# google/TensorNetwork

Measured on NVIDIA H100. Metric: pairwise contractions/s, higher is better.
Workload: dtype bf16

## Files before the change

### include/tnb200.h

```cpp
#ifndef TNB200_H_
#define TNB200_H_

#include <stdint.h>

#if defined(TNB200_BUILD)
#define TNB200_API __attribute__((visibility("default")))
#else
#define TNB200_API
#endif

#ifdef __cplusplus
extern "C" {
#endif

#define TNB200_MAX_NDIM 16
#define TNB200_ABI_VERSION 1

typedef enum {
  TNB200_OK = 0,
  TNB200_ERR_INVALID = -1,
  TNB200_ERR_DTYPE = -2,
  TNB200_ERR_CUDA = -3,
  TNB200_ERR_UNSUPPORTED = -4,
  TNB200_ERR_NOCONV = -5
// ... 76 lines not shown
                     int32_t axis1, int32_t axis2, void* stream);
TNB200_API int32_t tnb200_diagflat(const tnb200_tensor_t* a, const tnb200_tensor_t* c, int64_t k,
                        void* stream);

TNB200_API int32_t tnb200_svd(const tnb200_tensor_t* a, const tnb200_tensor_t* u, const tnb200_tensor_t* s,
                   const tnb200_tensor_t* vh, int32_t* info_dev, void* stream);
TNB200_API int32_t tnb200_svd_truncation_count(const tnb200_tensor_t* s, int64_t max_singular_values,
                                    int32_t use_error, double max_truncation_error,
                                    int32_t relative, int64_t* keep_dev, void* stream);

TNB200_API int32_t tnb200_eigh(const tnb200_tensor_t* a, const tnb200_tensor_t* w, const tnb200_tensor_t* v,
                               int32_t* info_dev, void* stream);

TNB200_API int32_t tnb200_arnoldi_orth(const tnb200_tensor_t* v, int32_t j, const tnb200_tensor_t* w, void* h_dev,
                                       void* stream);

TNB200_API int32_t tnb200_qr(const tnb200_tensor_t* a, const tnb200_tensor_t* q, const tnb200_tensor_t* r,
                  int32_t non_negative_diagonal, void* stream);

TNB200_API int32_t tnb200_lu_factor(const tnb200_tensor_t* a, const tnb200_tensor_t* lu, int32_t* piv_dev,
                                    int32_t* info_dev, void* stream);
TNB200_API int32_t tnb200_inv(const tnb200_tensor_t* a, const tnb200_tensor_t* x, int32_t* info_dev, void* stream);

TNB200_API int32_t tnb200_blocksparse_tensordot(const void* a_data, const void* b_data, void* c_data,
                                     int32_t dtype, int32_t nsect, const int64_t* dims_dev,
                                     const int64_t* a_map_dev, const int64_t* a_off_dev,
                                     const int64_t* b_map_dev, const int64_t* b_off_dev,
                                     const int64_t* c_map_dev, const int64_t* c_off_dev,
                                     int64_t max_m, int64_t max_n, int32_t conj_b, void* stream);

TNB200_API int32_t tnb200_svd_batched(const void* a_data, int32_t dtype, int32_t nprob, const int64_t* dims_dev,
                                      const int64_t* a_off_dev, void* u_data, const int64_t* u_off_dev, void* s_data,
                                      const int64_t* s_off_dev, void* vh_data, const int64_t* vh_off_dev,
                                      int64_t max_m, int64_t max_n, int32_t* status_dev, void* stream);

TNB200_API int32_t tnb200_blocksparse_maps(int32_t nlegs, const int64_t* dims, const int64_t* charges_dev, const int64_t* leg_off,
                                           const int32_t* order, int32_t partition, int32_t split, int64_t modulus, int64_t shift,
                                           int32_t nbins, const int64_t* tables_dev, int64_t nnz, int64_t* map_dev, void* stream);

TNB200_API int32_t tnb200_gather(const void* src, const int64_t* idx_dev, void* dst, int64_t n, int32_t dtype,
                                 int32_t scatter, void* stream);

typedef struct {
  tnb200_tensor_t a, b, c;
  int32_t naxes, nbatch;
  int32_t axes_a[TNB200_MAX_NDIM], axes_b[TNB200_MAX_NDIM];
  int32_t batch_a[TNB200_MAX_NDIM], batch_b[TNB200_MAX_NDIM];
  int32_t dep_a, dep_b;
} tnb200_chain_step_t;
TNB200_API int32_t tnb200_chain_create(int32_t nsteps, const tnb200_chain_step_t* steps, int32_t* first_unsupported,
                                       void** handle);
TNB200_API int32_t tnb200_chain_launch(void* handle, void* stream);
TNB200_API int32_t tnb200_chain_destroy(void* handle);

TNB200_API int32_t tnb200_thin_run_create(int32_t nsteps, const tnb200_chain_step_t* steps, int32_t* first_unsupported,
                                          void** handle);
TNB200_API int32_t tnb200_thin_run_launch(void* handle, void* stream);
TNB200_API int32_t tnb200_thin_run_destroy(void* handle);

#ifdef __cplusplus
}
#endif
#endif
```

### tensornetwork_b200/_lib.py

```python
import ctypes
import os

MAX_NDIM = 16
LIB_PATH = os.path.join(os.path.dirname(os.path.abspath(__file__)), "lib", "libtnb200.so")

F64, F32, F16, BF16, C64, C128, I32, I64, BOOL = range(9)
OK, ERR_INVALID, ERR_DTYPE, ERR_CUDA, ERR_UNSUPPORTED, ERR_NOCONV = 0, -1, -2, -3, -4, -5
ADD, SUB, MUL, DIV, POW = range(5)
CONJ, SQRT, ABS, NEG, EXP, LOG, SIN, COS, SIGN, REAL, IMAG = range(11)
LT, LE, GT, GE = range(4)
CONJ_A, CONJ_B = 1, 2
MATH_DEFAULT, MATH_STRICT, MATH_SIMT = 0 << 4, 1 << 4, 2 << 4


class TensorDesc(ctypes.Structure):
  _fields_ = [("data", ctypes.c_void_p), ("dtype", ctypes.c_int32), ("ndim", ctypes.c_int32),
              ("shape", ctypes.c_int64 * MAX_NDIM), ("stride", ctypes.c_int64 * MAX_NDIM)]


class ChainStep(ctypes.Structure):
  _fields_ = [("a", TensorDesc), ("b", TensorDesc), ("c", TensorDesc), ("naxes", ctypes.c_int32), ("nbatch", ctypes.c_int32),
              ("axes_a", ctypes.c_int32 * MAX_NDIM), ("axes_b", ctypes.c_int32 * MAX_NDIM),
              ("batch_a", ctypes.c_int32 * MAX_NDIM), ("batch_b", ctypes.c_int32 * MAX_NDIM),
              ("dep_a", ctypes.c_int32), ("dep_b", ctypes.c_int32)]


_P = ctypes.POINTER(TensorDesc)
_i32, _i64, _u64, _dbl, _vp = (ctypes.c_int32, ctypes.c_int64, ctypes.c_uint64, ctypes.c_double,
                               ctypes.c_void_p)
_pi32 = ctypes.POINTER(ctypes.c_int32)

SIGNATURES = {
    "tnb200_last_error": (ctypes.c_char_p, []),
    "tnb200_abi_version": (_i32, []),
    "tnb200_device_info": (_i32, [_pi32, _pi32, _pi32, ctypes.POINTER(_i64)]),
    "tnb200_last_kernel": (ctypes.c_char_p, []),
    "tnb200_launch_count": (_i64, []),
    "tnb200_tensordot": (_i32, [_P, _P, _P, _i32, _pi32, _pi32, _i32, _pi32, _pi32, _i32, _vp]),
    "tnb200_copy": (_i32, [_P, _P, _i32, _vp]),
    "tnb200_binary": (_i32, [_i32, _P, _P, _P, _vp]),
    "tnb200_unary": (_i32, [_i32, _P, _P, _vp]),
    "tnb200_affine_inplace": (_i32, [_P, _dbl, _dbl, _dbl, _dbl, _vp]),
    "tnb200_scale_by_device_scalar": (_i32, [_P, _vp, _i32, _i32, _vp]),
    "tnb200_axpy": (_i32, [_P, _P, _dbl, _dbl, _vp, _dbl, _vp]),
    "tnb200_fill": (_i32, [_P, _dbl, _dbl, _vp]),
    "tnb200_compare": (_i32, [_i32, _P, _P, _P, _vp]),
    "tnb200_index_update": (_i32, [_P, _P, _dbl, _dbl, _vp, _i32, _P, _vp]),
    "tnb200_eye": (_i32, [_P, _i64, _vp]),
    "tnb200_randn": (_i32, [_P, _u64, _vp]),
    "tnb200_uniform": (_i32, [_P, _dbl, _dbl, _u64, _vp]),
    "tnb200_norm": (_i32, [_P, _vp, _vp]),
    "tnb200_dot": (_i32, [_P, _P, _i32, _vp, _vp]),
    "tnb200_sum": (_i32, [_P, _P, _i32, _pi32, _vp]),
    "tnb200_trace": (_i32, [_P, _P, _i64, _i32, _i32, _vp]),
    "tnb200_diagflat": (_i32, [_P, _P, _i64, _vp]),
    "tnb200_svd": (_i32, [_P, _P, _P, _P, _vp, _vp]),
    "tnb200_svd_truncation_count": (_i32, [_P, _i64, _i32, _dbl, _i32, _vp, _vp]),
    "tnb200_eigh": (_i32, [_P, _P, _P, _vp, _vp]),
    "tnb200_arnoldi_orth": (_i32, [_P, _i32, _P, _vp, _vp]),
    "tnb200_qr": (_i32, [_P, _P, _P, _i32, _vp]),
    "tnb200_lu_factor": (_i32, [_P, _P, _vp, _vp, _vp]),
    "tnb200_inv": (_i32, [_P, _P, _vp, _vp]),
    "tnb200_blocksparse_maps": (_i32, [_i32, _vp, _vp, _vp, _vp, _i32, _i32, _i64, _i64, _i32, _vp, _i64, _vp, _vp]),
    "tnb200_svd_batched": (_i32, [_vp, _i32, _i32, _vp, _vp, _vp, _vp, _vp, _vp, _vp, _vp, _i64, _i64, _vp, _vp]),
    "tnb200_gather": (_i32, [_vp, _vp, _vp, _i64, _i32, _i32, _vp]),
    "tnb200_blocksparse_tensordot": (_i32, [_vp, _vp, _vp, _i32, _i32, _vp, _vp, _vp, _vp, _vp,
                                            _vp, _vp, _i64, _i64, _i32, _vp]),
    "tnb200_chain_create": (_i32, [_i32, ctypes.POINTER(ChainStep), _pi32, ctypes.POINTER(_vp)]),
    "tnb200_chain_launch": (_i32, [_vp, _vp]),
    "tnb200_chain_destroy": (_i32, [_vp]),
    "tnb200_thin_run_create": (_i32, [_i32, ctypes.POINTER(ChainStep), _pi32, ctypes.POINTER(_vp)]),
    "tnb200_thin_run_launch": (_i32, [_vp, _vp]),
    "tnb200_thin_run_destroy": (_i32, [_vp]),
}

_lib = None


def load(path=None):
  global _lib
  if _lib is not None:
    return _lib
  path = path or os.environ.get("TNB200_LIB", LIB_PATH)
  if not os.path.exists(path):
    raise OSError("libtnb200.so not found at {} — build it with "
                  "`python -m tensornetwork_b200.build` (there is no CPU fallback)".format(path))
  lib = ctypes.CDLL(path)
  for name, (res, args) in SIGNATURES.items():
    fn = getattr(lib, name)
    fn.restype = res
    fn.argtypes = args
  if lib.tnb200_abi_version() != 1:
    raise OSError("libtnb200.so ABI version mismatch")
  _lib = lib
  return lib


def set_lib(obj):
  global _lib
  _lib = obj


class Tnb200Error(RuntimeError):
  pass


def check(rc):
  if rc == 0:
    return
  msg = _lib.tnb200_last_error()
  msg = msg.decode() if isinstance(msg, bytes) else str(msg)
  if rc == ERR_INVALID:
    raise ValueError(msg)
  if rc == ERR_DTYPE:
    raise TypeError(msg)
  if rc == ERR_UNSUPPORTED:
    raise NotImplementedError(msg)
  raise Tnb200Error("tnb200 status {}: {}".format(rc, msg))
```

### tensornetwork_b200/csrc/gemm.cuh

```cuda
#pragma once
#include "common.cuh"

namespace tnb {

struct OperandView {
  const void* ptr = nullptr;
  int nF = 0, nK = 0;
  int64_t fe[4] = {1, 1, 1, 1}, fs[4] = {0, 0, 0, 0};
  int64_t ke[4] = {1, 1, 1, 1}, ks[4] = {0, 0, 0, 0};
  int64_t sb = 0;
  bool simple() const { return nF <= 1 && nK <= 1; }
  int64_t f_stride() const { return nF ? fs[nF - 1] : 0; }
  int64_t k_stride() const { return nK ? ks[nK - 1] : 0; }
};

struct GemmProblem {
  int dtype = 0;
  int64_t M = 0, N = 0, K = 0, batch = 1;
  OperandView A, B;
  void* C = nullptr; int64_t c_sm = 0, c_sn = 0, c_sb = 0;
  bool conjA = false, conjB = false;
  int math = 0;
  bool swapped = false;
};

int gemm_wgmma(const GemmProblem& p, cudaStream_t st);
int gemm_dmma_f64(const GemmProblem& p, cudaStream_t st);
int gemm_chain_create(int nsteps, const GemmProblem* probs, const int* dep_a, const int* dep_b, int* first_unsupported,
                      void** handle);
int gemm_chain_launch(void* handle, cudaStream_t st);
int gemm_chain_destroy(void* handle);
bool tma_view_ok(int dtype, const OperandView& v, int64_t ext_f, int64_t ext_k, int64_t batch);

}
```

### tensornetwork_b200/csrc/gemm_wgmma.cu

```cuda
#include "gemm.cuh"
#include "wgmma.cuh"
#include <cuda.h>
#include <mutex>
#include <vector>

namespace tnb {

__device__ __forceinline__ uint32_t smem_u32(const void* p) { return (uint32_t)__cvta_generic_to_shared(p); }

__device__ __forceinline__ void mbar_init(uint32_t bar, uint32_t count) {
  asm volatile("mbarrier.init.shared::cta.b64 [%0], %1;" ::"r"(bar), "r"(count));
}
__device__ __forceinline__ void mbar_expect_tx(uint32_t bar, uint32_t bytes) {
  asm volatile("mbarrier.arrive.expect_tx.shared::cta.b64 _, [%0], %1;" ::"r"(bar), "r"(bytes) : "memory");
}
__device__ __forceinline__ void mbar_arrive(uint32_t bar) {
  asm volatile("mbarrier.arrive.shared::cta.b64 _, [%0];" ::"r"(bar) : "memory");
}
__device__ __forceinline__ void mbar_wait(uint32_t bar, uint32_t parity) {
  uint32_t done = 0;
#pragma unroll 1
  for (uint32_t it = 0; it < (1u << 28); ++it) {
    asm volatile(
        "{\n\t.reg .pred p;\n\t"
// ... 54 lines not shown
}

struct TcParams {
  int64_t M, N, K, batch;
  int BN, num_kb, stages, out_kind;
  int64_t tiles_m, tiles_n, num_tiles;
  int a_mn, b_mn;
  uint32_t a_fe, a_ke, b_fe, b_ke;
  void* C; int64_t c_sm, c_sb;
  int64_t c_cs;
  int vec_ok;
};

constexpr int kBM = 128;
constexpr int kRowBytes = 128;
constexpr int kThreads = 384;

struct alignas(64) ChainStepDev {
  CUtensorMap tmA, tmB, tmC;
  TcParams p;
  int dep_a, dep_b;
  uint32_t need_a, need_b;
  int tiles_per_sample;
};
struct ChainSeg { long long tile0; int step, sample0, nsamples, pad; };
struct ChainParams {
  const ChainStepDev* steps;
  const ChainSeg* segs;
  uint32_t* done;
  long long num_tiles;
  int nsegs, batch, stages, stage_bytes;
};
constexpr int kConsumerWarps = 8;
constexpr int kChainBN16 = 256, kChainBN32 = 128;
constexpr int kBoxBytes = 64 * 128;
constexpr int kChainStageHalf = 2 * kBoxBytes;

struct KernelArgs {
  CUtensorMap tmA, tmB;
  TcParams p;
  ChainParams cp;
  int stage_bytes;
};

__device__ __forceinline__ uint32_t ld_acquire_u32(const uint32_t* p) {
  uint32_t v;
  asm volatile("ld.acquire.gpu.global.u32 %0, [%1];" : "=r"(v) : "l"(p) : "memory");
  return v;
}
__device__ __forceinline__ void red_release_add_u32(uint32_t* p, uint32_t v) {
  asm volatile("red.release.gpu.global.add.u32 [%0], %1;" ::"l"(p), "r"(v) : "memory");
}
#ifdef TNB200_CHAIN_PHASES
constexpr int kPhases = 6;
constexpr int kPhaseCtas = 1024;
__device__ unsigned long long g_chain_phase[kPhaseCtas * kPhases];
__device__ __forceinline__ unsigned long long phase_clock() {
  unsigned long long t;
  asm volatile("mov.u64 %0, %%globaltimer;" : "=l"(t)::"memory");
  return t;
}
#define TNB_PHASE(...) __VA_ARGS__
#define TNB_PHASE_ADD(slot, v) (g_chain_phase[blockIdx.x * kPhases + (slot)] += (v))
#else
#define TNB_PHASE(...)
#endif

__device__ __forceinline__ void chain_wait(const uint32_t* ctr, uint32_t need) {
#pragma unroll 1
  for (uint32_t it = 0; it < (1u << 24); ++it) {
    if (ld_acquire_u32(ctr) >= need) return;
    __nanosleep(64);
  }
  __trap();
}

struct Tile {
  const TcParams* p;
  const CUtensorMap *ma, *mb;
  const ChainStepDev* sd;
  int bi, mi, ni, step;
  bool live;
};
template <bool CHAIN>
__device__ __forceinline__ void decode_tile(const KernelArgs& a, long long tile, int rank, int& cursor, Tile& t) {
  if (!CHAIN) {
    uint32_t x = (uint32_t)tile;
    const uint32_t tn = (uint32_t)a.p.tiles_n, tm = (uint32_t)a.p.tiles_m;
    t.ni = (int)(x % tn); x /= tn;
    t.mi = (int)(x % tm);
    t.bi = (int)(x / tm);
    t.p = &a.p; t.ma = &a.tmA; t.mb = &a.tmB; t.sd = nullptr; t.step = 0;
    t.live = true;
  } else {
    const ChainParams& cp = a.cp;
    while (cursor + 1 < cp.nsegs && tile >= cp.segs[cursor + 1].tile0) ++cursor;
    const ChainSeg sg = cp.segs[cursor];
    const ChainStepDev* sd = cp.steps + sg.step;
    uint32_t local = (uint32_t)(tile - sg.tile0);
    const uint32_t tn = (uint32_t)sd->p.tiles_n, tm = (uint32_t)sd->p.tiles_m, pm = (tm + 1) / 2;
    t.ni = (int)(local % tn); local /= tn;
    t.mi = 2 * (int)(local % pm) + rank;
    t.bi = sg.sample0 + (int)(local / pm);
    t.step = sg.step;
    t.p = &sd->p; t.ma = &sd->tmA; t.mb = &sd->tmB; t.sd = sd;
    t.live = (uint32_t)t.mi < tm;
  }
// ... 16 lines not shown
    for (int i = 0; i < 4; ++i) {
      const int k = kc * 4 + i;
      const uint32_t addr = src + (uint32_t)k * 128u + (uint32_t)((((m >> 2) ^ (k & 7)) << 4) | ((m & 3) << 2));
      asm volatile("ld.shared.b32 %0, [%1];" : "=r"(v[i]) : "r"(addr) : "memory");
    }
    asm volatile("st.shared.v4.b32 [%0], {%1, %2, %3, %4};" ::"r"(dst), "r"(v[0]), "r"(v[1]), "r"(v[2]), "r"(v[3]) : "memory");
  }
  asm volatile("fence.proxy.async.shared::cta;" ::: "memory");
}

template <int KIND, int BN, int TA, int TB>
__device__ __forceinline__ void mma_k(float* d, uint64_t a, uint64_t b, uint32_t acc) {
  if constexpr (KIND == 2) {
    if constexpr (BN == 64) wgmma_n64_tf32(d, a, b, acc);
    else if constexpr (BN == 128) wgmma_n128_tf32(d, a, b, acc);
    else wgmma_n256_tf32(d, a, b, acc);
  } else if constexpr (KIND == 0) {
    if constexpr (BN == 64) wgmma_n64_bf16<TA, TB>(d, a, b, acc);
    else if constexpr (BN == 128) wgmma_n128_bf16<TA, TB>(d, a, b, acc);
    else wgmma_n256_bf16<TA, TB>(d, a, b, acc);
  } else {
    if constexpr (BN == 64) wgmma_n64_f16<TA, TB>(d, a, b, acc);
    else if constexpr (BN == 128) wgmma_n128_f16<TA, TB>(d, a, b, acc);
    else wgmma_n256_f16<TA, TB>(d, a, b, acc);
  }
}

template <bool PAIR>
__device__ __forceinline__ void release_slot(uint32_t bar) {
  if constexpr (PAIR) { mbar_arrive_cluster(bar, 0); mbar_arrive_cluster(bar, 1); }
  else mbar_arrive(bar);
}

__device__ __forceinline__ void drainloop(int S, uint32_t bar_base, int num_kb, int lane, int& s, uint32_t& ph) {
#pragma unroll 1
  for (int kb = 0; kb < num_kb; ++kb) {
    mbar_wait(bar_base + 8u * s, ph);
    __syncwarp();
    if (lane == 0) release_slot<true>(bar_base + 8u * (S + s));
    if (++s == S) { s = 0; ph ^= 1; }
  }
}

template <int KIND, int BN, int TA, int TB, bool PAIR>
__device__ __forceinline__ void mainloop(float* d, uint8_t* smem, int stage_bytes, int S, uint32_t bar_base, int num_kb,
                                         int a_mn, int b_mn, int wg, int ctid, int lane, int& s, uint32_t& ph) {
  constexpr int BK = kRowBytes / (KIND == 2 ? 4 : 2);
  constexpr uint32_t a_lbo = TA ? BK * kRowBytes : 16u, b_lbo = TB ? BK * kRowBytes : 16u;
  constexpr uint32_t a_kstep = TA ? 16u * kRowBytes : 32u, b_kstep = TB ? 16u * kRowBytes : 32u;
  int prev = -1;
  for (int kb = 0; kb < num_kb; ++kb) {
    TNB_PHASE(const unsigned long long tw = phase_clock();)
    mbar_wait(bar_base + 8u * s, ph);
    TNB_PHASE(if (ctid == 0) TNB_PHASE_ADD(1, phase_clock() - tw);)
    const uint32_t sa = smem_u32(smem + (size_t)s * stage_bytes);
    if (KIND == 2 && (a_mn || b_mn)) {
      transpose_stage_tf32(sa, a_mn, b_mn, BN, ctid);
      consumers_sync();
    }
    const uint32_t sa_wg = sa + (uint32_t)wg * 64u * kRowBytes;
    const uint32_t sb = sa + kBM * kRowBytes;
    wg_fence();
#pragma unroll
    for (int k = 0; k < 4; ++k)
      mma_k<KIND, BN, TA, TB>(d, gmma_desc(sa_wg + k * a_kstep, a_lbo, 1024u), gmma_desc(sb + k * b_kstep, b_lbo, 1024u),
                              (kb > 0 || k > 0) ? 1u : 0u);
    wg_commit();
    if (prev >= 0) {
      wg_wait<1>();
      __syncwarp();
      if (lane == 0) release_slot<PAIR>(bar_base + 8u * (S + prev));
    }
    prev = s;
    if (++s == S) { s = 0; ph ^= 1; }
  }
  wg_wait<0>();
  __syncwarp();
  if (lane == 0) release_slot<PAIR>(bar_base + 8u * (S + prev));
}

__device__ __forceinline__ void store_one(const TcParams& p, int64_t off, float v) {
  if (p.out_kind == 2) ((float*)p.C)[off] = v;
  else if (p.out_kind == 0) ((__nv_bfloat16*)p.C)[off] = __float2bfloat16_rn(v);
  else ((__half*)p.C)[off] = __float2half_rn(v);
}
__device__ __forceinline__ void store_pair(const TcParams& p, int64_t off, float v0, float v1) {
  if (p.out_kind == 2) *(float2*)((float*)p.C + off) = make_float2(v0, v1);
  else if (p.out_kind == 0) *(__nv_bfloat162*)((__nv_bfloat16*)p.C + off) = __floats2bfloat162_rn(v0, v1);
  else *(__half2*)((__half*)p.C + off) = __floats2half2_rn(v0, v1);
}

template <int KIND, int BN, bool CHAIN>
__global__ void __launch_bounds__(kThreads, 1)
gemm_wgmma_kernel(const __grid_constant__ KernelArgs args) {
  constexpr int ES = KIND == 2 ? 4 : 2;
  constexpr int BK = kRowBytes / ES;
  constexpr int CHUNK = kRowBytes / ES;
  constexpr int A_BYTES = kBM * kRowBytes;
  constexpr int B_BYTES = BN * kRowBytes;
  extern __shared__ __align__(1024) uint8_t smem_raw[];
  uint8_t* smem = (uint8_t*)(((uintptr_t)smem_raw + 1023) & ~(uintptr_t)1023);
  const int STAGE_BYTES = args.stage_bytes;
  const int S = CHAIN ? args.cp.stages : args.p.stages;
  const long long num_tiles = CHAIN ? args.cp.num_tiles : args.p.num_tiles;
  constexpr int STAGE_HALF = kChainStageHalf;
  const uint32_t staging = smem_u32(smem + (size_t)S * STAGE_BYTES);
  uint64_t* bars = (uint64_t*)(smem + (size_t)S * STAGE_BYTES + (CHAIN ? 2 * STAGE_HALF : 0));
// ... 51 lines not shown
        if (lane == 0) {
          TNB_PHASE(const unsigned long long tw = phase_clock();)
          const ChainStepDev* sd = t.sd;
          if (sd->dep_a >= 0) chain_wait(args.cp.done + (size_t)sd->dep_a * args.cp.batch + t.bi, sd->need_a);
          if (sd->dep_b >= 0) chain_wait(args.cp.done + (size_t)sd->dep_b * args.cp.batch + t.bi, sd->need_b);
          TNB_PHASE(TNB_PHASE_ADD(0, phase_clock() - tw);)
        }
        __syncwarp();
        asm volatile("fence.proxy.async;" ::: "memory");
      }
      int k_in = 0, k_out = 0;
      for (int kb = 0; kb < num_kb; ++kb) {
        mbar_wait(empty_bar(s), ph ^ 1);
        const uint32_t full = full_bar(s);
        if (lane == 0) mbar_expect_tx(full, tx_bytes);
        __syncwarp();
        if (mine) {
          const uint32_t dst = smem_u32(smem + (size_t)s * STAGE_BYTES) + dst_off;
          const int x0 = mn ? f_in : k_in, x1 = mn ? k_in : f_in, x2 = mn ? k_out : f_out, x3 = mn ? f_out : k_out;
          if (CHAIN && !is_a) tma_load_5d_pair(dst, map, full, x0, x1, x2, x3, t.bi);
          else                tma_load_5d(dst, map, full, x0, x1, x2, x3, t.bi);
        }
        k_in += BK;
        if (ke && (uint32_t)k_in >= ke) { k_in = 0; ++k_out; }
        if (++s == S) { s = 0; ph ^= 1; }
      }
    }
  } else if (warp >= 4) {
    const int ctid = threadIdx.x - 128;
    const int wg = ctid >> 7;
    const int wt = ctid & 127;
    int s = 0; uint32_t ph = 0;
    uint32_t eph = 0;
    int cursor = 0;
    float d[BN / 2];
    for (long long tile = first; tile < num_tiles; tile += step) {
      Tile t;
      decode_tile<CHAIN>(args, tile, rank, cursor, t);
      const TcParams& p = *t.p;
      const int a_mn = p.a_mn, b_mn = p.b_mn, num_kb = p.num_kb;
      if (CHAIN && !t.live) {
        drainloop(S, bar_base, num_kb, lane, s, ph);
        continue;
      }
      TNB_PHASE(const unsigned long long tk = phase_clock();)
      if constexpr (KIND == 2) {
        mainloop<KIND, BN, 0, 0, CHAIN>(d, smem, STAGE_BYTES, S, bar_base, num_kb, a_mn, b_mn, wg, ctid, lane, s, ph);
      } else {
        if (a_mn && b_mn) mainloop<KIND, BN, 1, 1, CHAIN>(d, smem, STAGE_BYTES, S, bar_base, num_kb, a_mn, b_mn, wg, ctid, lane, s, ph);
        else if (a_mn) mainloop<KIND, BN, 1, 0, CHAIN>(d, smem, STAGE_BYTES, S, bar_base, num_kb, a_mn, b_mn, wg, ctid, lane, s, ph);
        else if (b_mn) mainloop<KIND, BN, 0, 1, CHAIN>(d, smem, STAGE_BYTES, S, bar_base, num_kb, a_mn, b_mn, wg, ctid, lane, s, ph);
        else mainloop<KIND, BN, 0, 0, CHAIN>(d, smem, STAGE_BYTES, S, bar_base, num_kb, a_mn, b_mn, wg, ctid, lane, s, ph);
      }
      TNB_PHASE(const unsigned long long te = phase_clock(); if (ctid == 0) TNB_PHASE_ADD(2, te - tk);)
      const int r0 = (wt >> 5) * 16 + (lane >> 2);
      if constexpr (CHAIN) {
        constexpr int J_PER_PASS = BN / 8 * STAGE_HALF / (4 * kBoxBytes);
        const uint32_t half = staging + (uint32_t)wg * STAGE_HALF;
#pragma unroll
        for (int pass = 0; pass < 4 * kBoxBytes / STAGE_HALF; ++pass) {
          mbar_wait(freed_bar(wg), eph ^ 1);
#pragma unroll
          for (int jj = 0; jj < J_PER_PASS; ++jj) {
            const int j = pass * J_PER_PASS + jj;
            const uint32_t colb = (uint32_t)(8 * j + 2 * (lane & 3)) * ES - (uint32_t)pass * STAGE_HALF / 64;
#pragma unroll
            for (int h = 0; h < 2; ++h) {
              const uint32_t r = (uint32_t)(r0 + 8 * h);
              const uint32_t addr = half + (colb >> 7) * kBoxBytes + r * 128u + ((((colb >> 4) & 7) ^ (r & 7)) << 4) + (colb & 15);
              const float v0 = d[4 * j + 2 * h], v1 = d[4 * j + 2 * h + 1];
              if constexpr (KIND == 2) {
                asm volatile("st.shared.v2.f32 [%0], {%1, %2};" ::"r"(addr), "f"(v0), "f"(v1) : "memory");
              } else {
                uint32_t u;
                if constexpr (KIND == 0) { __nv_bfloat162 x = __floats2bfloat162_rn(v0, v1); u = *(uint32_t*)&x; }
                else { __half2 x = __floats2half2_rn(v0, v1); u = *(uint32_t*)&x; }
                asm volatile("st.shared.b32 [%0], %1;" ::"r"(addr), "r"(u) : "memory");
              }
            }
          }
          asm volatile("fence.proxy.async.shared::cta;" ::: "memory");
          __syncwarp();
          if (lane == 0) mbar_arrive(staged_bar(wg));
          eph ^= 1;
        }
        TNB_PHASE(if (ctid == 0) { TNB_PHASE_ADD(3, phase_clock() - te); TNB_PHASE_ADD(5, 1); })
        continue;
      }
      const int64_t row0 = (int64_t)t.mi * kBM + wg * 64 + r0;
      const int64_t n0 = (int64_t)t.ni * BN + 2 * (lane & 3);
      const int64_t cb = (int64_t)t.bi * p.c_sb;
#pragma unroll
      for (int h = 0; h < 2; ++h) {
        const int64_t row = row0 + 8 * h;
        if (row < p.M) {
#pragma unroll
          for (int j = 0; j < BN / 8; ++j) {
            const int64_t col = n0 + 8 * j;
            const float v0 = d[4 * j + 2 * h], v1 = d[4 * j + 2 * h + 1];
            if (p.c_cs == 1) {
              const int64_t off = cb + row * p.c_sm + col;
              if (p.vec_ok && col + 1 < p.N) store_pair(p, off, v0, v1);
              else {
                if (col < p.N) store_one(p, off, v0);
                if (col + 1 < p.N) store_one(p, off + 1, v1);
              }
            } else {
              const int64_t off = cb + row * p.c_sm + col * p.c_cs;
              if (col < p.N) store_one(p, off, v0);
              if (col + 1 < p.N) store_one(p, off + p.c_cs, v1);
            }
          }
        }
      }
    }
    TNB_PHASE(if (ctid == 0) TNB_PHASE_ADD(4, phase_clock() - t_start);)
  } else if (CHAIN && warp == 1 && lane == 0) {
    int cursor = 0;
    uint32_t sph = 0;
    for (long long tile = first; tile < num_tiles; tile += step) {
      Tile t;
      decode_tile<CHAIN>(args, tile, rank, cursor, t);
      if (!t.live) continue;
      const CUtensorMap* mc = &t.sd->tmC;
#pragma unroll 1
      for (int pass = 0; pass < 4 * kBoxBytes / STAGE_HALF; ++pass) {
#pragma unroll 1
        for (int wg = 0; wg < 2; ++wg) {
          mbar_wait(staged_bar(wg), sph);
          for (int b = 0; b < STAGE_HALF / kBoxBytes; ++b) {
            const int box = pass * (STAGE_HALF / kBoxBytes) + b;
            tma_store_3d(mc, staging + (uint32_t)(wg * STAGE_HALF + b * kBoxBytes), t.ni * BN + box * (128 / ES),
                         t.mi * kBM + wg * 64, t.bi);
          }
          bulk_commit();
          bulk_wait_read_all();
          mbar_arrive(freed_bar(wg));
        }
        sph ^= 1;
      }
      bulk_wait_all();
      asm volatile("fence.proxy.async.global;" ::: "memory");
      red_release_add_u32(args.cp.done + (size_t)t.step * args.cp.batch + t.bi, 1u);
    }
  }
  if constexpr (CHAIN) cluster_sync();
}

typedef CUresult (*EncodeTiledFn)(CUtensorMap*, CUtensorMapDataType, cuuint32_t, void*, const cuuint64_t*,
                                  const cuuint64_t*, const cuuint32_t*, const cuuint32_t*, CUtensorMapInterleave,
                                  CUtensorMapSwizzle, CUtensorMapL2promotion, CUtensorMapFloatOOBfill);
static EncodeTiledFn get_encode() {
  static EncodeTiledFn fn = nullptr;
  static std::once_flag once;
  std::call_once(once, []() {
    void* p = nullptr;
    cudaDriverEntryPointQueryResult q;
    if (cudaGetDriverEntryPoint("cuTensorMapEncodeTiled", &p, cudaEnableDefault, &q) == cudaSuccess &&
        q == cudaDriverEntryPointSuccess)
      fn = (EncodeTiledFn)p;
  });
  return fn;
}

static int es_of(int dt) { return dt == TNB200_F32 ? 4 : 2; }
static int kind_of(int dt) { return dt == TNB200_BF16 ? 0 : (dt == TNB200_F16 ? 1 : 2); }

static int view_major(int dtype, const OperandView& v, int64_t ext_f, int64_t ext_k, int64_t batch) {
  if (dtype != TNB200_F32 && dtype != TNB200_F16 && dtype != TNB200_BF16) return -1;
// ... 168 lines not shown
  if (e != cudaSuccess) { set_error("wgmma: cannot raise dynamic smem: %s", cudaGetErrorString(e)); return TNB200_ERR_CUDA; }
  return 0;
}

int gemm_wgmma(const GemmProblem& g, cudaStream_t st) {
  if (g.dtype != TNB200_F32 && g.dtype != TNB200_F16 && g.dtype != TNB200_BF16) return TNB200_ERR_UNSUPPORTED;
  if (g.conjA || g.conjB) return TNB200_ERR_UNSUPPORTED;
  if (!g.swapped && g.c_sn != 1 && g.N > 1) return TNB200_ERR_UNSUPPORTED;
  if (g.swapped && g.c_sm != 1 && g.M > 1) return TNB200_ERR_UNSUPPORTED;
  if (g.M >= (1LL << 31) || g.N >= (1LL << 31) || g.K >= (1LL << 31)) return TNB200_ERR_UNSUPPORTED;
  if (!tma_view_ok(g.dtype, g.A, g.M, g.K, g.batch) || !tma_view_ok(g.dtype, g.B, g.N, g.K, g.batch))
    return TNB200_ERR_UNSUPPORTED;
  if (g.M <= 64 && g.N >= 128 && !g.swapped) {
    GemmProblem t = g;
    t.swapped = true;
    t.M = g.N; t.N = g.M; t.A = g.B; t.B = g.A;
    t.c_sm = g.c_sn; t.c_sn = g.c_sm;
    return gemm_wgmma(t, st);
  }
  KernelArgs args;
  memset(&args, 0, sizeof(args));
  {
    TcPrep prep;
    int rc = tc_prepare(g, false, prep);
    if (rc) return rc;
    args.tmA = prep.tmA; args.tmB = prep.tmB; args.p = prep.p; args.stage_bytes = prep.stage_bytes;
  }
  const int kind = kind_of(g.dtype);
  KernelFn fn = kernel_of(kind, args.p.BN, false);
  static bool attr_set[3][3] = {};
  const int bi = args.p.BN == 64 ? 0 : (args.p.BN == 128 ? 1 : 2);
  if (!attr_set[kind][bi]) {
    int rc = raise_smem(fn);
    if (rc) return rc;
    attr_set[kind][bi] = true;
  }
  const int64_t sms = num_sms();
  const int64_t grid = args.p.num_tiles < sms ? args.p.num_tiles : sms;
  fn<<<(unsigned)grid, kThreads, smem_of(args.p.stages, args.stage_bytes), st>>>(args);
  TNB_LAUNCH_CHECK();
  count_launch();
  set_kernel_name(kind == 0 ? "wgmma_bf16" : (kind == 1 ? "wgmma_f16" : "wgmma_tf32"));
  return 0;
}

struct ChainHandle {
  ChainStepDev* d_steps = nullptr;
  ChainSeg* d_segs = nullptr;
  uint32_t* d_done = nullptr;
  KernelArgs args;
  int kind = 0, nsteps = 0;
  size_t smem = 0, done_bytes = 0;
  unsigned grid = 0;
};

struct PairLaunch {
  cudaLaunchAttribute attr;
  cudaLaunchConfig_t cfg;
  PairLaunch(unsigned grid, size_t smem, cudaStream_t st) {
    memset(&attr, 0, sizeof(attr));
    attr.id = cudaLaunchAttributeClusterDimension;
    attr.val.clusterDim.x = 2; attr.val.clusterDim.y = 1; attr.val.clusterDim.z = 1;
    memset(&cfg, 0, sizeof(cfg));
    cfg.gridDim = dim3(grid); cfg.blockDim = dim3(kThreads); cfg.dynamicSmemBytes = smem; cfg.stream = st;
    cfg.attrs = &attr; cfg.numAttrs = 1;
  }
  PairLaunch(const PairLaunch&) = delete;
};

int gemm_chain_create(int nsteps, const GemmProblem* probs, const int* dep_a, const int* dep_b, int* first_unsupported,
                      void** handle) {
  *handle = nullptr;
  if (nsteps < 1) return TNB200_ERR_INVALID;
  auto reject = [&](int i, int rc) { if (first_unsupported) *first_unsupported = i; return rc; };
  for (int i = 0; i < nsteps; ++i) {
    const GemmProblem& g = probs[i];
    if (g.M < 128 || g.N < 128 || g.batch != probs[0].batch || g.dtype != probs[0].dtype)
      return reject(i, TNB200_ERR_UNSUPPORTED);
  }
  const int dtype = probs[0].dtype;
  const int64_t batch = probs[0].batch;
  std::vector<ChainStepDev> steps(nsteps);
  int max_stage = 0;
  std::vector<int64_t> step_bytes(nsteps), out_bytes(nsteps);
  for (int i = 0; i < nsteps; ++i) {
    const GemmProblem& g = probs[i];
    if (g.conjA || g.conjB || g.swapped) return reject(i, TNB200_ERR_UNSUPPORTED);
    if (g.dtype != TNB200_F32 && g.dtype != TNB200_F16 && g.dtype != TNB200_BF16) return reject(i, TNB200_ERR_UNSUPPORTED);
    if (g.c_sn != 1 || g.M >= (1LL << 31) || g.N >= (1LL << 31) || g.K >= (1LL << 31)) return reject(i, TNB200_ERR_UNSUPPORTED);
    if (dep_a[i] >= i || dep_b[i] >= i) return TNB200_ERR_INVALID;
    TcPrep prep;
    int rc = tc_prepare(g, true, prep);
    if (rc) return reject(i, rc);
    ChainStepDev& sd = steps[i];
    memset(&sd, 0, sizeof(sd));
    rc = encode_output(&sd.tmC, g);
    if (rc) return reject(i, rc);
    sd.tmA = prep.tmA; sd.tmB = prep.tmB; sd.p = prep.p;
    sd.dep_a = dep_a[i]; sd.dep_b = dep_b[i];
    sd.tiles_per_sample = (int)(prep.p.tiles_m * prep.p.tiles_n);
    if (prep.stage_bytes > max_stage) max_stage = prep.stage_bytes;
    step_bytes[i] = (g.M * g.K + g.N * g.K + g.M * g.N) * es_of(dtype);
    out_bytes[i] = g.M * g.N * es_of(dtype);
  }
  for (int i = 0; i < nsteps; ++i) {
    if (steps[i].dep_a >= 0) steps[i].need_a = (uint32_t)steps[steps[i].dep_a].tiles_per_sample;
    if (steps[i].dep_b >= 0) steps[i].need_b = (uint32_t)steps[steps[i].dep_b].tiles_per_sample;
  }
  const int kind = kind_of(dtype);
  KernelFn fn = kernel_of(kind, 0, true);
  {
    static bool attr_set[3] = {};
    if (!attr_set[kind]) {
      int rc = raise_smem(fn);
      if (rc) return rc;
      attr_set[kind] = true;
    }
  }
  const int staging = 2 * kChainStageHalf;
  int stages = (227 * 1024 - 1024 - staging - 256) / max_stage;
  if (stages > 8) stages = 8;
  if (stages < 2) return TNB200_ERR_UNSUPPORTED;
  const size_t smem = smem_of(stages, max_stage) + staging + 4 * 8;
  int clusters = 0;
  {
    PairLaunch pl(2 * num_sms(), smem, nullptr);
    if (cudaOccupancyMaxActiveClusters(&clusters, (void*)fn, &pl.cfg) != cudaSuccess) {
      cudaGetLastError();
      clusters = 0;
    }
  }
  if (clusters < 1) return TNB200_ERR_UNSUPPORTED;
  std::vector<int> pps(nsteps);
  for (int i = 0; i < nsteps; ++i) pps[i] = (int)(steps[i].p.tiles_n * ((steps[i].p.tiles_m + 1) / 2));
  auto env_int = [](const char* name, int dflt) { const char* e = getenv(name); return e ? atoi(e) : dflt; };
  int min_pps = pps[0];
  for (int i = 1; i < nsteps; ++i) if (pps[i] < min_pps) min_pps = pps[i];
  if (batch * min_pps < clusters && !env_int("TNB200_CHAIN_FORCE", 0))
    return TNB200_ERR_UNSUPPORTED;
  int l2 = 0;
  {
    int dev = 0;
    if (cudaGetDevice(&dev) != cudaSuccess || cudaDeviceGetAttribute(&l2, cudaDevAttrL2CacheSize, dev) != cudaSuccess) {
      cudaGetLastError();
      l2 = 0;
    }
  }
  int g_wave = 1;
  std::vector<int> last_reader(nsteps, -1);
  for (int i = 0; i < nsteps; ++i) {
    for (const int d : {dep_a[i], dep_b[i]}) {
      if (d < 0) continue;
      last_reader[d] = i;
      int64_t gap = 0;
      for (int j = d; j < i; ++j) gap += pps[j];
      const int g = (int)((clusters + gap - 1) / gap);
      if (g > g_wave) g_wave = g;
    }
  }
  int64_t live_bytes = 0;
  for (int i = 0; i < nsteps; ++i) {
    int64_t live = step_bytes[i];
    for (int j = 0; j < i; ++j)
      if (last_reader[j] > i && dep_a[i] != j && dep_b[i] != j) live += out_bytes[j];
    if (live > live_bytes) live_bytes = live;
  }
  const int g_l2 = (int)(l2 / live_bytes);
  int G = env_int("TNB200_CHAIN_G", g_wave > g_l2 ? g_wave : g_l2);
  if (G < 1) G = 1;
  const int64_t rounds = (batch + G - 1) / G;
  std::vector<ChainSeg> segs;
  long long tile0 = 0;
  for (int64_t r = 0; r < rounds; ++r) {
    const int64_t r0 = batch * r / rounds, r1 = batch * (r + 1) / rounds;
    for (int i = 0; i < nsteps; ++i) {
      ChainSeg sg;
      sg.tile0 = tile0; sg.step = i; sg.sample0 = (int)r0; sg.nsamples = (int)(r1 - r0); sg.pad = 0;
      segs.push_back(sg);
      tile0 += (long long)(r1 - r0) * pps[i];
    }
  }
  ChainHandle* h = new ChainHandle();
  h->kind = kind;
  h->nsteps = nsteps;
  h->done_bytes = sizeof(uint32_t) * (size_t)nsteps * (size_t)batch;
  cudaError_t e = cudaMalloc(&h->d_steps, sizeof(ChainStepDev) * steps.size());
  if (e == cudaSuccess) e = cudaMalloc(&h->d_segs, sizeof(ChainSeg) * segs.size());
  if (e == cudaSuccess) e = cudaMalloc(&h->d_done, h->done_bytes);
  if (e == cudaSuccess) e = cudaMemcpy(h->d_steps, steps.data(), sizeof(ChainStepDev) * steps.size(), cudaMemcpyHostToDevice);
  if (e == cudaSuccess) e = cudaMemcpy(h->d_segs, segs.data(), sizeof(ChainSeg) * segs.size(), cudaMemcpyHostToDevice);
  if (e != cudaSuccess) {
    set_error("chain: device table allocation failed: %s", cudaGetErrorString(e));
    cudaFree(h->d_steps); cudaFree(h->d_segs); cudaFree(h->d_done);
    delete h;
    return TNB200_ERR_CUDA;
  }
  memset(&h->args, 0, sizeof(h->args));
  ChainParams& cp = h->args.cp;
  cp.steps = h->d_steps; cp.segs = h->d_segs; cp.done = h->d_done;
  cp.num_tiles = tile0; cp.nsegs = (int)segs.size(); cp.batch = (int)batch;
  cp.stages = stages; cp.stage_bytes = max_stage;
  h->args.stage_bytes = max_stage;
  h->smem = smem;
  h->grid = (unsigned)(2 * (tile0 < clusters ? tile0 : clusters));
  *handle = h;
  return 0;
}

int gemm_chain_launch(void* handle, cudaStream_t st) {
  ChainHandle* h = (ChainHandle*)handle;
  if (!h) return TNB200_ERR_INVALID;
  TNB_CHECK_CUDA(cudaMemsetAsync(h->d_done, 0, h->done_bytes, st));
  PairLaunch pl(h->grid, h->smem, st);
  TNB_CHECK_CUDA(cudaLaunchKernelEx(&pl.cfg, kernel_of(h->kind, 0, true), h->args));
  count_launch();
  set_kernel_name(h->kind == 2 ? "wgmma_chain_tf32" : "wgmma_chain_16");
  return 0;
}

int gemm_chain_destroy(void* handle) {
  ChainHandle* h = (ChainHandle*)handle;
  if (!h) return 0;
  cudaFree(h->d_steps); cudaFree(h->d_segs); cudaFree(h->d_done);
  delete h;
  return 0;
}

}

#ifdef TNB200_CHAIN_PHASES
extern "C" TNB200_API int32_t tnb200_chain_phases(unsigned long long* out, int32_t reset) {
  if (cudaMemcpyFromSymbol(out, tnb::g_chain_phase, sizeof(tnb::g_chain_phase)) != cudaSuccess) return TNB200_ERR_CUDA;
  if (reset) {
    void* p = nullptr;
    if (cudaGetSymbolAddress(&p, tnb::g_chain_phase) != cudaSuccess || cudaMemset(p, 0, sizeof(tnb::g_chain_phase)) != cudaSuccess)
      return TNB200_ERR_CUDA;
  }
  return 0;
}
#endif
```

### tensornetwork_b200/csrc/tensordot.cu

```cuda
#include "gemm.cuh"
#include <algorithm>
#include <vector>

namespace tnb {

int copy_strided(const tnb200_tensor_t* src, const tnb200_tensor_t* dst, int conj, cudaStream_t st);
int tensordot_thin(int dt, const void* A, const void* B, void* C, const ModeList& mB, const ModeList& mM,
                   const ModeList& mN, const ModeList& mK, bool allow_tf32, cudaStream_t st);
int tensordot_skinny(int dt, const void* A, const void* B, void* C, const ModeList& mB, const ModeList& mM,
                     const ModeList& mN, const ModeList& mK, cudaStream_t st);
int thin_run_create(int dt, int nsteps, const ModeList* mB, const ModeList* mM, const ModeList* mN, const ModeList* mK,
                    const void* const* A, const void* const* B, void* const* C, const int* dep_a, const int* dep_b,
                    int* bad, void** handle);
int thin_run_launch(void* handle, cudaStream_t st);
int thin_run_destroy(void* handle);

template <typename T>
struct SimtParams {
  const T* A; const T* B; T* C;
  DevModes mB;
  DevModes mM;
  DevModes mN;
  DevModes mK;
  int64_t M, N, K, batch;
// ... 397 lines not shown
    void* pk[2] = {nullptr, nullptr};
    int64_t pitch[2] = {0, 0};
    auto packed = [&](int w, const OperandView* split, OperandView& v) -> int {
      if (!pk[w]) {
        int rc = pack_operand(dt, w ? b->data : a->data, w, gB, w ? gN : gM, L.ko, &pk[w], &pitch[w], st);
        if (rc) return rc;
      }
      const int64_t F = w ? N : M;
      v = OperandView();
      v.ptr = pk[w]; v.nF = 1; v.fe[0] = F; v.fs[0] = pitch[w]; v.sb = F * pitch[w];
      v.nK = split ? split->nK : 1;
      int64_t s = 1;
      for (int i = v.nK - 1; i >= 0; --i) { v.ke[i] = split ? split->ke[i] : K; v.ks[i] = s; s *= v.ke[i]; }
      return 0;
    };
    int rc = 0;
    for (int attempt = 0; attempt < 2; ++attempt) {
      const bool keepA = attempt == 0 && L.inA, keepB = attempt == 0 && L.inB;
      if (!keepA) rc = packed(0, keepB ? &g.B : nullptr, g.A);
      if (rc == 0 && !keepB) rc = packed(1, keepA ? &g.A : nullptr, g.B);
      if (rc) break;
      rc = dt == TNB200_F64 ? gemm_dmma_f64(g, st) : gemm_wgmma(g, st);
      if (rc != TNB200_ERR_UNSUPPORTED || !(L.inA || L.inB)) break;
    }
    ws_free(pk[0], st);
    ws_free(pk[1], st);
    if (rc != TNB200_ERR_UNSUPPORTED) return rc;
  }
  ModeList gK = mK;
  merge_modes(gK, 2);
  return dispatch_simt(dt, a->data, b->data, c->data, gB, gM, gN, gK, conjA, conjB, st);
}

extern "C" int32_t tnb200_chain_create(int32_t nsteps, const tnb200_chain_step_t* steps, int32_t* first_unsupported,
                                       void** handle) {
  TNB_REQUIRE(nsteps >= 1 && steps && handle, TNB200_ERR_INVALID, "chain: bad arguments");
  *handle = nullptr;
  if (first_unsupported) *first_unsupported = -1;
  std::vector<GemmProblem> probs((size_t)nsteps);
  std::vector<int> da((size_t)nsteps), db((size_t)nsteps);
  for (int i = 0; i < nsteps; ++i) {
    const tnb200_chain_step_t& s = steps[i];
    int rc = plan_inplace_gemm(s, probs[i]);
    if (rc) { if (first_unsupported) *first_unsupported = i; return rc; }
    da[i] = s.dep_a; db[i] = s.dep_b;
    TNB_REQUIRE(s.dep_a < i && s.dep_b < i, TNB200_ERR_INVALID, "chain: step %d depends on a later step", i);
    TNB_REQUIRE(s.dep_a < 0 || steps[s.dep_a].c.data == s.a.data, TNB200_ERR_INVALID, "chain: dep_a of step %d does not produce its operand", i);
    TNB_REQUIRE(s.dep_b < 0 || steps[s.dep_b].c.data == s.b.data, TNB200_ERR_INVALID, "chain: dep_b of step %d does not produce its operand", i);
  }
  return gemm_chain_create(nsteps, probs.data(), da.data(), db.data(), first_unsupported, handle);
}
extern "C" int32_t tnb200_chain_launch(void* handle, void* stream) { return gemm_chain_launch(handle, (cudaStream_t)stream); }
extern "C" int32_t tnb200_chain_destroy(void* handle) { return gemm_chain_destroy(handle); }

extern "C" int32_t tnb200_thin_run_create(int32_t nsteps, const tnb200_chain_step_t* steps, int32_t* first_unsupported,
                                          void** handle) {
  TNB_REQUIRE(nsteps >= 1 && steps && handle, TNB200_ERR_INVALID, "thin run: bad arguments");
  *handle = nullptr;
  if (first_unsupported) *first_unsupported = -1;
  std::vector<ModeList> mB((size_t)nsteps), mM((size_t)nsteps), mN((size_t)nsteps), mK((size_t)nsteps);
  std::vector<const void*> A((size_t)nsteps), B((size_t)nsteps);
  std::vector<void*> C((size_t)nsteps);
  std::vector<int> da((size_t)nsteps), db((size_t)nsteps);
  for (int i = 0; i < nsteps; ++i) {
    const tnb200_chain_step_t& s = steps[i];
    int rc = build_modes(&s.a, &s.b, &s.c, s.naxes, s.axes_a, s.axes_b, s.nbatch, s.batch_a, s.batch_b, mB[i], mM[i],
                         mN[i], mK[i]);
    if (rc) { if (first_unsupported) *first_unsupported = i; return rc; }
    TNB_REQUIRE(s.dep_a < i && s.dep_b < i, TNB200_ERR_INVALID, "thin run: step %d depends on a later step", i);
    merge_modes(mB[i], 3); merge_modes(mM[i], 2); merge_modes(mN[i], 2); merge_modes(mK[i], 2);
    A[i] = s.a.data; B[i] = s.b.data; C[i] = s.c.data;
    da[i] = s.dep_a; db[i] = s.dep_b;
  }
  int bad = -1;
  const int rc = thin_run_create(steps[0].a.dtype, nsteps, mB.data(), mM.data(), mN.data(), mK.data(), A.data(), B.data(),
                                 C.data(), da.data(), db.data(), &bad, handle);
  if (rc && first_unsupported) *first_unsupported = bad;
  return rc;
}
extern "C" int32_t tnb200_thin_run_launch(void* handle, void* stream) {
  TNB_REQUIRE(handle, TNB200_ERR_INVALID, "thin run: null handle");
  return thin_run_launch(handle, (cudaStream_t)stream);
}
extern "C" int32_t tnb200_thin_run_destroy(void* handle) { return thin_run_destroy(handle); }
```

Measured before the change: 1.155 million.

## Derive chain round count from L2 budget and dependency gap

Changes how the fused GEMM chain splits the batch into rounds. Before, it took the maximum of a wave-based and an L2-capacity group size. Now the round count is sized so that live intermediates fit in half of L2, and it is capped by the minimum producer-consumer gap measured in cluster waves. The goal is to keep intermediates L2-resident while leaving enough tiles between dependent steps to avoid stalls. It also adds a query API exposing the chosen round size and slack, and splits the first-k-block wait into its own profiling phase; the plan may yield more rounds and lower per-round parallelism.

```diff
diff --git a/include/tnb200.h b/include/tnb200.h
--- a/include/tnb200.h
+++ b/include/tnb200.h
@@ -152,6 +152,7 @@
                                        void** handle);
 TNB200_API int32_t tnb200_chain_launch(void* handle, void* stream);
 TNB200_API int32_t tnb200_chain_destroy(void* handle);
+TNB200_API int32_t tnb200_chain_plan(const void* handle, int32_t* round, double* slack_waves);
 
 TNB200_API int32_t tnb200_thin_run_create(int32_t nsteps, const tnb200_chain_step_t* steps, int32_t* first_unsupported,
                                           void** handle);
diff --git a/tensornetwork_b200/_lib.py b/tensornetwork_b200/_lib.py
--- a/tensornetwork_b200/_lib.py
+++ b/tensornetwork_b200/_lib.py
@@ -69,6 +69,7 @@
     "tnb200_chain_create": (_i32, [_i32, ctypes.POINTER(ChainStep), _pi32, ctypes.POINTER(_vp)]),
     "tnb200_chain_launch": (_i32, [_vp, _vp]),
     "tnb200_chain_destroy": (_i32, [_vp]),
+    "tnb200_chain_plan": (_i32, [_vp, _pi32, ctypes.POINTER(_dbl)]),
     "tnb200_thin_run_create": (_i32, [_i32, ctypes.POINTER(ChainStep), _pi32, ctypes.POINTER(_vp)]),
     "tnb200_thin_run_launch": (_i32, [_vp, _vp]),
     "tnb200_thin_run_destroy": (_i32, [_vp]),
diff --git a/tensornetwork_b200/csrc/gemm.cuh b/tensornetwork_b200/csrc/gemm.cuh
--- a/tensornetwork_b200/csrc/gemm.cuh
+++ b/tensornetwork_b200/csrc/gemm.cuh
@@ -30,6 +30,7 @@
                       void** handle);
 int gemm_chain_launch(void* handle, cudaStream_t st);
 int gemm_chain_destroy(void* handle);
+int gemm_chain_plan(const void* handle, int* round, double* slack_waves);
 bool tma_view_ok(int dtype, const OperandView& v, int64_t ext_f, int64_t ext_k, int64_t batch);
 
 }
diff --git a/tensornetwork_b200/csrc/gemm_wgmma.cu b/tensornetwork_b200/csrc/gemm_wgmma.cu
--- a/tensornetwork_b200/csrc/gemm_wgmma.cu
+++ b/tensornetwork_b200/csrc/gemm_wgmma.cu
@@ -130,7 +130,7 @@
   asm volatile("red.release.gpu.global.add.u32 [%0], %1;" ::"l"(p), "r"(v) : "memory");
 }
 #ifdef TNB200_CHAIN_PHASES
-constexpr int kPhases = 6;
+constexpr int kPhases = 7;
 constexpr int kPhaseCtas = 1024;
 __device__ unsigned long long g_chain_phase[kPhaseCtas * kPhases];
 __device__ __forceinline__ unsigned long long phase_clock() {
@@ -253,7 +253,7 @@
   for (int kb = 0; kb < num_kb; ++kb) {
     TNB_PHASE(const unsigned long long tw = phase_clock();)
     mbar_wait(bar_base + 8u * s, ph);
-    TNB_PHASE(if (ctid == 0) TNB_PHASE_ADD(1, phase_clock() - tw);)
+    TNB_PHASE(if (ctid == 0) TNB_PHASE_ADD(kb == 0 ? 1 : 2, phase_clock() - tw);)
     const uint32_t sa = smem_u32(smem + (size_t)s * stage_bytes);
     if (KIND == 2 && (a_mn || b_mn)) {
       transpose_stage_tf32(sa, a_mn, b_mn, BN, ctid);
@@ -411,7 +411,7 @@
         else if (b_mn) mainloop<KIND, BN, 0, 1, CHAIN>(d, smem, STAGE_BYTES, S, bar_base, num_kb, a_mn, b_mn, wg, ctid, lane, s, ph);
         else mainloop<KIND, BN, 0, 0, CHAIN>(d, smem, STAGE_BYTES, S, bar_base, num_kb, a_mn, b_mn, wg, ctid, lane, s, ph);
       }
-      TNB_PHASE(const unsigned long long te = phase_clock(); if (ctid == 0) TNB_PHASE_ADD(2, te - tk);)
+      TNB_PHASE(const unsigned long long te = phase_clock(); if (ctid == 0) TNB_PHASE_ADD(3, te - tk);)
       const int r0 = (wt >> 5) * 16 + (lane >> 2);
       if constexpr (CHAIN) {
         constexpr int J_PER_PASS = BN / 8 * STAGE_HALF / (4 * kBoxBytes);
@@ -443,7 +443,7 @@
           if (lane == 0) mbar_arrive(staged_bar(wg));
           eph ^= 1;
         }
-        TNB_PHASE(if (ctid == 0) { TNB_PHASE_ADD(3, phase_clock() - te); TNB_PHASE_ADD(5, 1); })
+        TNB_PHASE(if (ctid == 0) { TNB_PHASE_ADD(4, phase_clock() - te); TNB_PHASE_ADD(6, 1); })
         continue;
       }
       const int64_t row0 = (int64_t)t.mi * kBM + wg * 64 + r0;
@@ -473,7 +473,7 @@
         }
       }
     }
-    TNB_PHASE(if (ctid == 0) TNB_PHASE_ADD(4, phase_clock() - t_start);)
+    TNB_PHASE(if (ctid == 0) TNB_PHASE_ADD(5, phase_clock() - t_start);)
   } else if (CHAIN && warp == 1 && lane == 0) {
     int cursor = 0;
     uint32_t sph = 0;
@@ -748,6 +748,8 @@
   int kind = 0, nsteps = 0;
   size_t smem = 0, done_bytes = 0;
   unsigned grid = 0;
+  int round = 0;
+  double slack = 0;
 };
 
 struct PairLaunch {
@@ -842,7 +844,7 @@
       l2 = 0;
     }
   }
-  int g_wave = 1;
+  int64_t min_gap = 0;
   std::vector<int> last_reader(nsteps, -1);
   for (int i = 0; i < nsteps; ++i) {
     for (const int d : {dep_a[i], dep_b[i]}) {
@@ -850,8 +852,7 @@
       last_reader[d] = i;
       int64_t gap = 0;
       for (int j = d; j < i; ++j) gap += pps[j];
-      const int g = (int)((clusters + gap - 1) / gap);
-      if (g > g_wave) g_wave = g;
+      if (min_gap == 0 || gap < min_gap) min_gap = gap;
     }
   }
   int64_t live_bytes = 0;
@@ -861,10 +862,16 @@
       if (last_reader[j] > i && dep_a[i] != j && dep_b[i] != j) live += out_bytes[j];
     if (live > live_bytes) live_bytes = live;
   }
-  const int g_l2 = (int)(l2 / live_bytes);
-  int G = env_int("TNB200_CHAIN_G", g_wave > g_l2 ? g_wave : g_l2);
-  if (G < 1) G = 1;
-  const int64_t rounds = (batch + G - 1) / G;
+  const int64_t budget = l2 / 2;
+  int64_t rounds = budget > 0 ? (batch * live_bytes + budget - 1) / budget : 1;
+  if (min_gap && rounds > batch * min_gap / clusters) rounds = batch * min_gap / clusters;
+  if (getenv("TNB200_CHAIN_G")) {
+    int G = env_int("TNB200_CHAIN_G", 1);
+    if (G < 1) G = 1;
+    rounds = (batch + G - 1) / G;
+  }
+  if (rounds < 1) rounds = 1;
+  if (rounds > batch) rounds = batch;
   std::vector<ChainSeg> segs;
   long long tile0 = 0;
   for (int64_t r = 0; r < rounds; ++r) {
@@ -899,7 +906,17 @@
   h->args.stage_bytes = max_stage;
   h->smem = smem;
   h->grid = (unsigned)(2 * (tile0 < clusters ? tile0 : clusters));
+  h->round = (int)((batch + rounds - 1) / rounds);
+  h->slack = min_gap ? (double)(batch / rounds) * (double)min_gap / clusters : 0.0;
   *handle = h;
+  return 0;
+}
+
+int gemm_chain_plan(const void* handle, int* round, double* slack_waves) {
+  const ChainHandle* h = (const ChainHandle*)handle;
+  if (!h) return TNB200_ERR_INVALID;
+  if (round) *round = h->round;
+  if (slack_waves) *slack_waves = h->slack;
   return 0;
 }
 
diff --git a/tensornetwork_b200/csrc/tensordot.cu b/tensornetwork_b200/csrc/tensordot.cu
--- a/tensornetwork_b200/csrc/tensordot.cu
+++ b/tensornetwork_b200/csrc/tensordot.cu
@@ -473,6 +473,9 @@
 }
 extern "C" int32_t tnb200_chain_launch(void* handle, void* stream) { return gemm_chain_launch(handle, (cudaStream_t)stream); }
 extern "C" int32_t tnb200_chain_destroy(void* handle) { return gemm_chain_destroy(handle); }
+extern "C" int32_t tnb200_chain_plan(const void* handle, int32_t* round, double* slack_waves) {
+  return gemm_chain_plan(handle, round, slack_waves);
+}
 
 extern "C" int32_t tnb200_thin_run_create(int32_t nsteps, const tnb200_chain_step_t* steps, int32_t* first_unsupported,
                                           void** handle) {
```

Measured after the change: 1.171 million, median of 6. 1.4% higher.
